# modelscope/FunCodec

Hardware: AMD Instinct MI355X
Metric: audio-seconds encoded+decoded per wall-sec, 16k-nq32ds640 (higher is better)
Workload: dtype f32; 1 GPU; BASELINE.json configs[1]: encodec 16k-nq32ds640 (57.6M, synthetic seeded checkpoint), run_mod=inference (encode + 32-stage RVQ + decode), 16 x 10 s utterances per GPU in micro-batches of 16, n_q=32; utterances_per_gpu=16, samples_per_utterance=160000, micro_batch=16, global_utterances=16, ranks_seen=1, parallelism=single GPU

## Files before the change

funcodec_amd/build.py:

```python
from __future__ import annotations

import concurrent.futures
import glob
import os
import shutil
import subprocess

HERE = os.path.dirname(os.path.abspath(__file__))
CSRC = os.path.join(HERE, "csrc")
LIB_PATH = os.path.join(HERE, "libfuncodec_amd.so")
OBJ_DIR = os.path.join(CSRC, "_obj")
HEADERS = ["kernels.h", "device_common.h", "conv_kernel.h", "laura_kernels.h", "seq_kernels.h", "stream_kernels.h", "ragged_kernels.h", "slots_kernels.h", os.path.join("..", "..", "include", "funcodec_amd.h")]


def sources():
    tiles = sorted(os.path.basename(p) for p in glob.glob(os.path.join(CSRC, "conv_tile*_*.hip")))
    heavy = [t for t in tiles if t.startswith("conv_tileq_") and "_m" not in t] + [t for t in tiles if t.endswith("_m01.hip")]
    rest = [t for t in tiles if t not in heavy]
    return heavy + ["kernels.hip", "laura_persist.hip", "laura_kernels.hip", "freq_kernels.hip", "seq_kernels.hip", "seqstream_kernels.hip", "stream_kernels.hip", "ragged_kernels.hip", "slots_kernels.hip", "engine.hip", "laura.hip"] + rest


def _hipcc() -> str:
    for cand in (os.environ.get("HIPCC"), shutil.which("hipcc"), "/opt/rocm/bin/hipcc"):
        if cand and os.path.exists(cand):
            return cand
    raise RuntimeError("hipcc not found")


def needs_build() -> bool:
    if not os.path.exists(LIB_PATH):
        return True
    t = os.path.getmtime(LIB_PATH)
    deps = [os.path.join(CSRC, s) for s in sources() + HEADERS]
    return any(os.path.exists(d) and os.path.getmtime(d) > t for d in deps)


def build(force: bool = False, verbose: bool = False) -> str:
    timeline = bool(os.environ.get("FC_TIMELINE"))
    out = LIB_PATH.replace(".so", "_timeline.so") if timeline else LIB_PATH
    defines = ["-DFC_TIMELINE", "-DFC_AB_KNOBS"] if timeline else []
    defines += ["-D" + f for f in os.environ.get("FC_BUILD_DEFINES", "").split()]
    if os.environ.get("FC_BUILD_OUT"):
        out = os.environ["FC_BUILD_OUT"]
    if not force and not defines and out == LIB_PATH and not needs_build():
        return LIB_PATH
    import hashlib
    hipcc = _hipcc()
    base = [hipcc, "--offload-arch=gfx950", "-O3", "-std=c++17", "-fPIC"] + defines
    tag = "".join(c if c.isalnum() else "_" for c in os.path.basename(out)) + "_" + hashlib.sha1(" ".join(base[1:]).encode()).hexdigest()[:10]
    obj_dir = os.path.join(OBJ_DIR, tag)
    os.makedirs(obj_dir, exist_ok=True)
    hdr_time = max(os.path.getmtime(os.path.join(CSRC, h)) for h in HEADERS if os.path.exists(os.path.join(CSRC, h)))

    def compile_one(src: str) -> str:
        obj = os.path.join(obj_dir, src.replace(".hip", ".o"))
        path = os.path.join(CSRC, src)
        if not force and os.path.exists(obj) and os.path.getmtime(obj) > max(os.path.getmtime(path), hdr_time):
            return obj
        cmd = base + ["-c", path, "-o", obj]
        if verbose:
            print(" ".join(cmd), flush=True)
        subprocess.run(cmd, check=True)
        return obj

    srcs = sources()
    with concurrent.futures.ThreadPoolExecutor(max_workers=min(len(srcs), os.cpu_count() or 4)) as ex:
        objs = list(ex.map(compile_one, srcs))
    tmp_out = f"{out}.{os.getpid()}.tmp"
    link = [hipcc, "--offload-arch=gfx950", "-shared", "-fPIC", "-o", tmp_out] + objs
    if verbose:
        print(" ".join(link), flush=True)
    subprocess.run(link, check=True)
# ... 7 lines not shown
```

funcodec_amd/csrc/engine.hip:

```cpp
#include <hip/hip_runtime.h>

#include <algorithm>
#include <array>
#include <cmath>
#include <cstdio>
#include <cstring>
#include <map>
#include <memory>
#include <string>
#include <vector>

#include "../../include/funcodec_amd.h"
#include "kernels.h"
#include "laura_kernels.h"
#include "ragged_kernels.h"
#include "seq_kernels.h"
#include "slots_kernels.h"
#include "stream_kernels.h"

namespace {

thread_local std::string g_err;

int fail(const std::string& msg) { g_err = msg; return 1; }
// ... 178 lines not shown
    ~Session() { drop_graphs(); }
};

struct fc_stream : Session {
    int enc_pushes = 0, dec_pushes = 0;
    int enc_frames = 0, dec_frames = 0;
    bool enc_done = false;
    bool broken = false;
};

struct fc_slots : Session {
    enum Phase : char { Idle, Running, Ended, Poisoned };
    std::vector<char> enc_phase, dec_phase;
    int enc_pushes = 0, dec_pushes = 0;
    std::vector<int32_t> push;
    std::vector<int32_t> enc_frames, dec_frames;
};

namespace {

hipEvent_t prof_event(fc_engine* e) {
    if (e->events_used == e->event_pool.size()) {
        hipEvent_t ev;
        if (hipEventCreate(&ev) != hipSuccess) return nullptr;
        e->event_pool.push_back(ev);
    }
    return e->event_pool[e->events_used++];
}

struct ProfSpan {
    fc_engine* e; hipStream_t st; int idx = -1;
    template <typename Cls>
    ProfSpan(fc_engine* e_, hipStream_t st_, bool live, Cls&& cls, double flops, double bytes) : e(e_), st(st_) {
        if (!e->profiling || !live) return;
        fc_engine::Span s; s.cls = e->prof_class(cls()); s.a = prof_event(e); s.b = prof_event(e); s.flops = flops; s.bytes = bytes;
        if (!s.a || !s.b) return;
        (void)hipEventRecord(s.a, st);
        e->spans.push_back(s);
        idx = (int)e->spans.size() - 1;
    }
    ~ProfSpan() { if (idx >= 0) (void)hipEventRecord(e->spans[idx].b, st); }
};

struct Ctx {
    fc_engine* e = nullptr;
    int B = 0;
    hipStream_t st = nullptr;
    char* base = nullptr;
    size_t cap = 0, off = 256;
    bool dry = false;
    int err = 0;
    bool dec_side = false, no_xq = false;
    int rate = 1;
    static constexpr size_t kTailSlack = 4096;
    int launches = 0, conv_launches = 0;
    double conv_flops = 0, conv_bytes = 0, lstm_flops = 0, rvq_flops = 0, attn_flops = 0;
    bool live() const { return !dry && !err; }
    void fail(const std::string& msg) {
        if (!err) { err = 1; g_err = msg; }
    }
    template <typename T>
    T* alloc(size_t n) {
        off = (off + 255) & ~(size_t)255;
        T* p = dry ? nullptr : (T*)(base + off);
        off += n * sizeof(T);
        if (!dry && off + kTailSlack > cap) { fail("workspace too small (sizes from fc_engine_workspace_bytes include 4 KiB of tail slack)"); return nullptr; }
        return p;
    }
    template <typename Enqueue>
    void launch(const char* what, const char* layer, Enqueue&& enqueue) {
        ++launches;
        if (live()) check(enqueue(), what, layer);
    }
    template <typename Cls, typename Enqueue>
    void launch(const char* what, const char* layer, Cls&& cls, double flops, double bytes, Enqueue&& enqueue) {
        ++launches;
        if (!live()) return;
        ProfSpan sp(e, st, true, cls, flops, bytes);
        check(enqueue(), what, layer);
    }
    template <typename Cls, typename Enqueue>
    void conv_launch(const char* what, const char* layer, Cls&& cls, double flops, double bytes, Enqueue&& enqueue) {
        ++conv_launches;
        launch(what, layer, cls, flops, bytes, enqueue);
    }
    void check(hipError_t er, const char* what, const char* layer) {
        if (er != hipSuccess) fail(std::string(what) + " launch failed" + (*layer ? std::string(" (") + layer + ")" : "") + ": " + hipGetErrorString(er));
    }
};

Ctx make_ctx(fc_engine* e, int B, void* ws, size_t ws_bytes, void* stream) {
    Ctx cx;
    cx.e = e; cx.B = B; cx.st = (hipStream_t)stream; cx.base = (char*)ws; cx.cap = ws_bytes;
    return cx;
}

Ctx dry_ctx(fc_engine* e, int B) {
    Ctx cx = make_ctx(e, B, nullptr, 0, nullptr);
    cx.dry = true;
    return cx;
}

template <typename T>
T* at(T* p, long long off) { return p ? p + off : nullptr; }

enum class Role { First, Shortcut, Block1, Block3, Resample, Last };
// ... 760 lines not shown
        cx.launch("halo rows", L.prefix.c_str(),
                  [&] { return fc::launch_halo_rows(halo_of->buf, cx.B, halo_of->F, halo_of->halo, halo_of->C, halo_of->T, 0, cx.st); });
}

Act run_conv(fc_engine* e, Ctx& cx, const ConvLayer& L, fc::Src s0, fc::Src s1, int elu, int Tin,
             float* out_override = nullptr, long long sB = 0, long long sM = 0, long long sT = 0) {
    const ConvGeom g = conv_geom(L, Tin);
    const bool has_prologue = (s0.used & 2) || s1.used || elu;
    int xq_Tp = 0;
    if ((L.Mpad / L.BM >= 3 || L.force_plain) && has_prologue) {
        const bool xq = !cx.no_xq && !s0.div && !out_override_blocks_xq(L) && fc::conv_xq_ok(L.cin, L.CC, L.gk, L.gstride, L.dil, L.BM, L.BN, L.row ? 1 : 0);
        const int padL_x = L.transposed ? 1 : g.padL, padR_x = L.transposed ? 1 : g.padR;
        const int Tp = padL_x + Tin + padR_x;
        float* tmp = xq ? cx.alloc<float>(fc::conv_xq_floats(cx.B, L.cin, Tp, L.BN, L.gstride, L.gk, L.dil))
                        : cx.alloc<float>((size_t)cx.B * L.cin * Tin);
        cx.launch("combine", L.prefix.c_str(), [&] {
            return xq ? fc::launch_combine_xq(s0, s1, elu, e->arch.elu_alpha, cx.B, L.cin, Tin, padL_x, padR_x, (L.transposed || L.zpadL >= 0) ? 1 : 0, tmp, cx.st)
                      : fc::launch_combine(s0, s1, elu, e->arch.elu_alpha, nullptr, cx.B, L.cin, Tin, Tin, tmp, (long long)L.cin * Tin, Tin, 1, cx.st);
        });
        s0 = fc::Src(); s0.ptr = tmp; s0.used = 1;
        s1 = fc::Src();
        elu = 0;
        if (xq) xq_Tp = Tp;
    }
    fc::ConvLaunch c = conv_launch_of(L, cx.B, Tin, g);
    c.s0 = s0; c.s1 = s1; c.elu = elu; c.alpha = e->arch.elu_alpha;
    c.xq_Tp = xq_Tp;
    Act out;
    out.C = L.cout; out.T = g.Tout;
    if (L.transposed) {
        c.Tout = Tin + 1; c.pad_zero = 1;
        c.up_r = L.stride; c.trimL = L.causal ? 0 : L.stride - L.stride / 2; c.Tfinal = g.Tout;
    } else {
        c.Tout = g.Tout;
        if (L.zpadL >= 0) c.pad_zero = 1;
    }
    if (out_override) {
        out.raw = out_override;
        c.out_sB = sB; c.out_sM = sM; c.out_sT = sT;
    } else {
        out.raw = cx.alloc<float>((size_t)cx.B * L.cout * g.Tout);
        c.out_sB = (long long)L.cout * g.Tout; c.out_sM = g.Tout; c.out_sT = 1;
    }
    c.out = out.raw;
    const int nblk = fc::conv_nblk(c);
    if (L.has_norm) {
        c.partials = cx.alloc<double>((size_t)cx.B * nblk * 2);
        out.aff = cx.alloc<float>((size_t)cx.B * L.cout * 2);
        out.normed = true;
    }
    const double fl = 2.0 * cx.B * (double)L.M * L.cin * L.gk * c.Tout;
    const double by = 4.0 * cx.B * ((double)L.cin * Tin * (s1.used ? 2 : 1) + (double)L.cout * g.Tout);
    cx.conv_flops += fl; cx.conv_bytes += by;
    cx.conv_launch("conv", L.prefix.c_str(), [&] { return conv_class(c); }, fl, by, [&] { return fc::launch_conv(c, cx.st); });
    conv_finish(e, cx, L, c.partials, nblk, (double)L.cout * g.count_T, out.aff);
    return out;
}

inline fc::Src src_of(const Act& a) { fc::Src s; s.ptr = a.raw; s.aff = a.aff; s.used = a.normed ? 3 : 1; s.ld = a.ld; return s; }

Act run_lstm(fc_engine* e, Ctx& cx, const LstmBlock& lb, const Act& in, int T, float* carried = nullptr, const fc::RagLen* steps = nullptr) {
    const int H = lb.H, B = cx.B, L = (int)lb.layers.size();
    float* xproj = cx.alloc<float>((size_t)T * B * 4 * H);
    run_conv(e, cx, lb.layers[0].inproj, src_of(in), fc::Src(), 0, T, xproj, (long long)4 * H, 1, (long long)B * 4 * H);
    static const int persist_env = fc::deploy_switch("FC_LSTM_PERSIST", 1);
    bool persist = false;
    if (!carried && persist_env && e->lstm_persist_ok) {
        const int key = B * 4096 + H;
        if (e->persist_checked_B != key) { e->persist_checked_val = fc::lstm_persist_supported(B, H, L, e->device); e->persist_checked_B = key; }
        persist = e->persist_checked_val;
    }
    const size_t BH = (size_t)B * H;
    float* state = carried ? carried : cx.alloc<float>(persist ? fc::lstm_persist_state_floats(B, H, T) : 3 * L * BH);
    Act y;
    y.C = H; y.T = T;
    y.raw = cx.alloc<float>((size_t)B * H * T);
    const double fl = 2.0 * B * (double)T * 4 * H * H * (2 * L - 1);
    cx.lstm_flops += fl;
    const double by = 4.0 * (4.0 * H * H * (2 * L - 1) + (double)T * B * 4.0 * H + (double)B * H * T);
    const float* w[FC_LSTM_MAX_LAYERS] = {nullptr};
    const float* bias[FC_LSTM_MAX_LAYERS] = {nullptr};
    for (int l = 0; l < L; ++l) { w[l] = l == 0 ? lb.layers[0].whh : lb.layers[l].wcat; bias[l] = lb.layers[l].bperm; }
    const char* pre = lb.prefix.c_str();
    ProfSpan sp(e, cx.st, cx.live(), [&] { return persist ? kLstmPersistClass : kLstmWaveClass; }, fl, by);
    if (!carried)
        cx.launch("lstm state clear", pre,
                  [&] { return fc::launch_zero_fill(state, persist ? fc::lstm_persist_clear_floats(B, H) : 3 * L * BH, cx.st); });
    if (persist) {
        cx.launch("lstm", pre, [&] { return fc::launch_lstm_persist(w[0], w[1], bias[1], xproj, state, y.raw, B, H, T, e->status_dev, cx.st); });
    } else {
        for (int s = 0; s < T + L - 1; ++s)
            cx.launch("lstm step", pre, [&] {
                return steps ? fc::launch_lstm_wave(w, bias, xproj, state, state + 2 * L * BH, y.raw, B, H, T, L, s, cx.st, steps->lens, steps->div, steps->mul)
                             : fc::launch_lstm_wave(w, bias, xproj, state, state + 2 * L * BH, y.raw, B, H, T, L, s, cx.st);
            });
    }
    if (carried && (T & 1))
        for (int l = 0; l < L; ++l)
            cx.launch("lstm carry", pre, [&] {
                return hipMemcpyAsync(state + (size_t)(2 * l + 1) * BH, state + (size_t)(2 * l) * BH, BH * sizeof(float), hipMemcpyDeviceToDevice, cx.st);
            });
    return y;
}

struct TfCache {
    float* base = nullptr;
// ... 167 lines not shown
}

void run_bottleneck(fc_engine* e, Ctx& cx, const Pass& p, bool dec, const Act& x, fc::Src* a0, fc::Src* a1) {
    const LstmBlock& lb = dec ? e->dec_lstm : e->enc_lstm;
    const TfBlock& tb = dec ? e->dec_tf : e->enc_tf;
    *a0 = src_of(x); *a1 = fc::Src();
    if (!has_seq(lb, tb)) return;
    Act y;
    switch (p.kind) {
        case Pass::Stream:
            if (tb.C) {
                const TfCache kv = tf_cache(*p.sess, dec, dec ? static_cast<const fc_stream*>(p.sess)->dec_frames : static_cast<const fc_stream*>(p.sess)->enc_frames);
                if (!cx.dry && kv.pos + x.T > p.sess->max_frames) { cx.fail("internal: a push past max_frames reached the transformer"); return; }
                y = run_transformer(e, cx, tb, x, x.T, &kv);
            } else {
                y = run_lstm(e, cx, lb, x, x.T, lstm_state(*p.sess, dec));
            }
            break;
        case Pass::Slots: {
            const fc::RagLen steps = ragged_len(cx, p);
            if (tb.C) {
                TfCache kv = tf_cache(*p.sess, dec, 0);
                kv.rows = true; kv.len = steps; kv.pos_dev = p.pos;
                if (p.host_push) { kv.host_len = p.host_push; kv.host_pos = p.host_push + 2 * cx.B; }
                kv.grid_bound = p.graphed;
                y = run_transformer(e, cx, tb, x, x.T, &kv);
            } else {
                y = run_lstm(e, cx, lb, x, x.T, lstm_state(*p.sess, dec), &steps);
            }
            break;
        }
        case Pass::Ragged:
        case Pass::Offline: y = run_seq(e, cx, lb, tb, x, x.T); break;
    }
    *a0 = src_of(y);
    if (e->arch.lstm_skip) *a1 = src_of(x);
}

void run_resblocks(fc_engine* e, Ctx& cx, const Pass& p, const fc_engine::Stage& S, fc::Src a0, fc::Src a1, int T, Act* sc, Act* b3) {
    for (const auto& R : S.res) {
        Act b1;
        if (p.kind == Pass::Offline && R.fused_head && !a0.div) {
            run_reshead(e, cx, R, a0, a1, T, sc, &b1);
        } else {
            *sc = walk_conv(e, cx, p, Role::Shortcut, R.shortcut, a0, a1, 0, T);
            b1 = walk_conv(e, cx, p, Role::Block1, R.block1, a0, a1, 1, T);
        }
        *b3 = walk_conv(e, cx, p, Role::Block3, R.block3, src_of(b1), fc::Src(), 1, b1.T);
        a0 = src_of(*sc); a1 = src_of(*b3);
    }
}

Act run_encoder(fc_engine* e, Ctx& cx, const Pass& p, fc::Src wav, int T) {
    cx.dec_side = false; cx.rate = 1; cx.no_xq = p.kind == Pass::Ragged;
    Act x = walk_conv(e, cx, p, Role::First, e->enc_first, wav, fc::Src(), 0, T);
    for (auto& S : e->enc_stages) {
        Act sc, b3;
        run_resblocks(e, cx, p, S, src_of(x), fc::Src(), x.T, &sc, &b3);
        x = walk_conv(e, cx, p, Role::Resample, S.resample, src_of(sc), src_of(b3), 1, sc.T);
        cx.rate *= S.resample.stride;
    }
    fc::Src a0, a1;
    run_bottleneck(e, cx, p, false, x, &a0, &a1);
    return walk_conv(e, cx, p, Role::Last, e->enc_last, a0, a1, 1, x.T);
}

Act run_decoder(fc_engine* e, Ctx& cx, const Pass& p, const float* z_bdt, int Tf) {
    fc::Src s; s.ptr = z_bdt; s.used = 1;
    cx.dec_side = true; cx.rate = 1; cx.no_xq = p.kind == Pass::Ragged;
    Act x = walk_conv(e, cx, p, Role::First, e->dec_first, s, fc::Src(), 0, Tf);
    fc::Src a0, a1;
    run_bottleneck(e, cx, p, true, x, &a0, &a1);
    int T = Tf;
    for (auto& S : e->dec_stages) {
        Act up = walk_conv(e, cx, p, Role::Resample, S.resample, a0, a1, 1, T);
        cx.rate *= S.resample.stride;
        Act sc, b3;
        run_resblocks(e, cx, p, S, src_of(up), fc::Src(), up.T, &sc, &b3);
        a0 = src_of(sc); a1 = src_of(b3);
        T = up.T;
    }
    return walk_conv(e, cx, p, Role::Last, e->dec_last, a0, a1, 1, T);
}



Act2 materialise2d(fc_engine* e, Ctx& cx, const ConvLayer& L, const Act2& x0, const Act2* x1, int elu, int pad) {
    const int B = cx.B, C = L.c2d;
    Act2 m;
    m.C = C; m.F = x0.F; m.T = x0.T; m.halo = x0.halo;
    m.buf = cx.alloc<float>((size_t)B * (m.F + 2 * m.halo) * C * m.T);
    const bool fuse_halo = !pad && halo_fuse_on() && m.F > m.halo;
    cx.launch("combine2d", L.prefix.c_str(), [&] {
        if (x0.halo < pad) return hipErrorInvalidValue;
        return fc::launch_combine2d(x0.buf, x0.aff, x0.halo, x1 ? x1->buf : nullptr, x1 ? x1->aff : nullptr, x1 ? x1->halo : 0, elu, e->arch.elu_alpha,
                                    B, m.F, C, m.T, m.buf, m.halo, cx.st, fuse_halo ? 1 : 0);
    });
    if (pad) cx.launch("halo rows", L.prefix.c_str(), [&] { return fc::launch_halo_rows_short(m.buf, B, m.F, m.halo, pad, C, m.T, cx.st); });
    else if (!fuse_halo) cx.launch("halo rows", L.prefix.c_str(), [&] { return fc::launch_halo_rows(m.buf, B, m.F, m.halo, C, m.T, 0, cx.st); });
    return m;
}

Act2 run_conv2d(fc_engine* e, Ctx& cx, const ConvLayer& L, Act2 x0, const Act2* x1, int elu, int out_halo) {
    const int B = cx.B, C = L.c2d, kf = L.kf, sf = L.sf;
    const int tot_f = (kf - 1) - (sf - 1), f_after = tot_f / 2, f_before = tot_f - f_after;
    const int Fo = (x0.F + tot_f - kf) / sf + 1;
    const ConvGeom g = conv_geom(L, x0.T);
    const int fpad = std::max(f_before, f_after);
    if (x0.F <= fpad) { x0 = materialise2d(e, cx, L, x0, x1, elu, fpad); x1 = nullptr; elu = 0; }
    bool mat;
    if (L.w_group) {
        static const int gmat = fc::ab_knob("FC_GCONV_MAT", 1);
        mat = gmat && kf >= 4 && x1;
    } else {
        static const int few_mat = fc::ab_knob("FC_FEWOUT_MAT", 1);
        const bool few_out = few_mat && L.cout <= 4 && L.stride == 1 && sf == 1 && (L.k == 3 || L.k == 5 || L.k == 7) && kf > 1;
        mat = (L.Mpad / L.BM >= 3 || few_out || L.force_plain) && (x0.normed || x1 || elu);
    }
    if (mat) { x0 = materialise2d(e, cx, L, x0, x1, elu, 0); x1 = nullptr; elu = 0; }
    Act2 o;
    o.C = L.cout; o.F = Fo; o.T = g.Tout; o.halo = out_halo;
    o.buf = cx.alloc<float>((size_t)B * (Fo + 2 * out_halo) * L.cout * g.Tout);
// ... 1439 lines not shown
    return cx.err;
}
}

int fc_freq_synthesis_size(const fc_engine* ce, int B, int C, int F, int Tp, int out_len, size_t* workspace_bytes) {
    fc_engine* e = const_cast<fc_engine*>(ce);
    if (freq_synthesis_check(e, B, C, F, Tp, out_len)) return 1;
    if (!workspace_bytes) return fail("null argument");
    Ctx cx = dry_ctx(e, B);
    if (freq_synthesis(e, cx, nullptr, nullptr, nullptr, Tp, out_len, nullptr, nullptr)) return 1;
    *workspace_bytes = cx.off + 4096;
    return 0;
}

int fc_freq_synthesis(fc_engine* e, const float* dec, const float* aff, const float* scale, int B, int C, int F, int Tp, int out_len, float* wav,
                      float* spec, void* workspace, size_t workspace_bytes, void* stream) {
    if (freq_synthesis_check(e, B, C, F, Tp, out_len)) return 1;
    if (!dec || !wav) return fail("bad argument");
    if (check_ready(e)) return 1;
    Ctx cx = make_ctx(e, B, workspace, workspace_bytes, stream);
    return freq_synthesis(e, cx, dec, aff, scale, Tp, out_len, wav, spec);
}

namespace {
fc::Src hook_src(const float* x, const float* aff, const float* div) {
    fc::Src s;
    s.ptr = x; s.aff = aff; s.div = div;
    s.used = x ? ((aff || div) ? 3 : 1) : 0;
    return s;
}
}

static int layer_src_check(const fc_engine* e, const char* prefix, const float* x0, const float* aff0, const float* div0, const float* x1,
                           const float* aff1, int B, int T, const ConvLayer** out) {
    if (!e || !prefix || !x0 || B <= 0 || T <= 0 || (aff1 && !x1) || (aff0 && div0)) return fail("bad argument");
    auto it = e->by_prefix.find(prefix);
    if (it == e->by_prefix.end()) return fail(std::string("unknown layer ") + prefix);
    const ConvLayer& L = *it->second;
    if (L.c2d > 0)
        return fail(std::string("layer ") + prefix + " is a 2-D layer of the STFT-domain codec: use fc_layer2d_forward");
    if (x1 && !L.dual) return fail("fc_layer_forward_src: " + L.prefix + " is planned for one source (its staging has no room for two)");
    if (div0 && &L != &e->enc_first) return fail("fc_layer_forward_src: div0 is the encoder's first conv's volume scale (" + e->enc_first.prefix + ")");
    *out = &L;
    return 0;
}

int fc_layer_forward_src(fc_engine* e, const char* prefix, const float* x0, const float* aff0, const float* div0, const float* x1,
                         const float* aff1, int B, int T, int apply_elu, float* y, void* workspace, size_t workspace_bytes, void* stream) {
    const ConvLayer* L = nullptr;
    if (layer_src_check(e, prefix, x0, aff0, div0, x1, aff1, B, T, &L)) return 1;
    if (!y) return fail("bad argument");
    if (check_ready(e)) return 1;
    Ctx cx = make_ctx(e, B, workspace, workspace_bytes, stream);
    Act o = run_conv(e, cx, *L, hook_src(x0, aff0, div0), hook_src(x1, aff1, nullptr), apply_elu, T);
    if (cx.err) return 1;
    HIP_TRY(fc::launch_combine(src_of(o), fc::Src(), 0, 1.f, nullptr, B, o.C, o.T, o.T, y, (long long)o.C * o.T, o.T, 1, cx.st));
    return 0;
}

int fc_layer_forward(fc_engine* e, const char* prefix, const float* x, int B, int T, int apply_elu, float* y,
                     void* workspace, size_t workspace_bytes, void* stream) {
    return fc_layer_forward_src(e, prefix, x, nullptr, nullptr, nullptr, nullptr, B, T, apply_elu, y, workspace, workspace_bytes, stream);
}

int fc_resblock_forward_src(fc_engine* e, const char* prefix, const float* x0, const float* aff0, const float* x1, const float* aff1, int B,
                            int T, float* y, void* workspace, size_t workspace_bytes, void* stream) {
    if (!e || !prefix || !x0 || !y || B <= 0 || T <= 0 || (aff1 && !x1)) return fail("bad argument");
    auto it = e->res_by_prefix.find(prefix);
    if (it == e->res_by_prefix.end()) return fail(std::string("unknown residual block ") + prefix);
    const fc_engine::ResBlock& R = *it->second;
    if (x1 && !R.shortcut.dual)
        return fail(std::string("fc_resblock_forward_src: block ") + prefix + " is planned for one source (its staging has no room for two)");
    if (check_ready(e)) return 1;
    Ctx cx = make_ctx(e, B, workspace, workspace_bytes, stream);
    fc_engine::Stage one;
    one.res.push_back(R);
    Act sc, b3;
    run_resblocks(e, cx, Pass(), one, hook_src(x0, aff0, nullptr), hook_src(x1, aff1, nullptr), T, &sc, &b3);
    if (cx.err) return 1;
    HIP_TRY(fc::launch_combine(src_of(sc), src_of(b3), 0, 1.f, nullptr, B, sc.C, T, T, y, (long long)sc.C * T, T, 1, cx.st));
    return 0;
}

int fc_resblock_forward(fc_engine* e, const char* prefix, const float* x, int B, int T, float* y, void* workspace,
                        size_t workspace_bytes, void* stream) {
    return fc_resblock_forward_src(e, prefix, x, nullptr, nullptr, nullptr, B, T, y, workspace, workspace_bytes, stream);
}

int fc_lstm_forward(fc_engine* e, const char* prefix, const float* x, int B, int T, float* y, void* workspace,
                    size_t workspace_bytes, void* stream) {
    if (check_ready(e)) return 1;
    if (!prefix || !x || !y || B <= 0 || T <= 0) return fail("bad argument");
    auto it = e->lstm_by_prefix.find(prefix);
    if (it == e->lstm_by_prefix.end()) return fail(std::string("unknown lstm ") + prefix);
    Ctx cx = make_ctx(e, B, workspace, workspace_bytes, stream);
    Act in; in.raw = const_cast<float*>(x); in.C = it->second->H; in.T = T;
    Act o = run_lstm(e, cx, *it->second, in, T);
    if (cx.err) return 1;
    fc::Src s1;
    if (e->arch.lstm_skip) s1 = src_of(in);
    HIP_TRY(fc::launch_combine(src_of(o), s1, 0, 1.f, nullptr, B, o.C, T, T, y, (long long)o.C * T, T, 1, cx.st));
    return 0;
}

int fc_seq_forward(fc_engine* e, const char* prefix, const float* x, int B, int T, float* y, void* workspace,
                   size_t workspace_bytes, void* stream) {
// ... 472 lines not shown
```

funcodec_amd/csrc/kernels.h:

```cpp
#pragma once
#include <hip/hip_runtime.h>
#include <stdint.h>
#include <stdio.h>
#include <stdlib.h>

#include <vector>

namespace fc {

inline int ab_knob(const char* name, int dflt) {
#ifdef FC_AB_KNOBS
    const char* v = getenv(name);
    return v ? atoi(v) : dflt;
#else
    if (getenv(name)) fprintf(stderr, "funcodec_amd: %s is set but ignored by this build (tuning knobs need FC_BUILD_DEFINES=FC_AB_KNOBS)\n", name);
    return dflt;
#endif
}

inline int deploy_switch(const char* name, int dflt) {
    const char* v = getenv(name);
    return v ? atoi(v) : dflt;
}

struct Src {
    const float* ptr = nullptr;
    const float* aff = nullptr;
    const float* div = nullptr;
    int used = 0;
    int ld = 0;
};

struct ConvLaunch {
    Src s0, s1;
    int elu = 0; float alpha = 1.f;
    const float* wt = nullptr;
    const float* bias = nullptr;
    const int* koff = nullptr;
    float* out = nullptr;
    long long out_sB = 0, out_sM = 0, out_sT = 1;
    int B = 0, Cin = 0, Tin = 0;
    int M = 0;
    int Tout = 0;
    int k = 1, stride = 1, padL = 0, padR = 0;
    int dil = 1;
    int pad_zero = 0;
    int up_r = 0, trimL = 0, Tfinal = 0;
    double* partials = nullptr;
    int BM = 128, BN = 128, CC = 2, nchunk = 1;
    int row = 0;
    int xq_Tp = 0;
    int Fo = 1;
    int affC = 0;
    long long in_sB0 = 0, in_sB1 = 0;
    long long out_sF = 0, part_sB0 = 0;
    int store_lo = 0, store_hi = 1 << 30;
    const float* w_plain = nullptr;
    float bias_host0 = 0.f;
};

int conv_nblk(const ConvLaunch& c);
bool conv_cout1_ok(const ConvLaunch& c);
bool conv_fewout_rows(const ConvLaunch& c);
void conv_fewout_name(const ConvLaunch& c, char* buf, size_t n);
size_t conv_lds_bytes(const ConvLaunch& c);
int conv_wbuf_floats(int k, int CC, int BM);
bool conv_quad(int CC);
size_t conv_pack_index(int k, int CC, int BM, int kk, int cl, int mm);
size_t conv_lds_bytes_for(int k, int stride, int dil, int CC, int BM, int BN, int Cin, int ntab, int row, int dma_rounds = -1);
bool conv_row_ok(int k, int stride, int dil, int CC, int BM, int BN, int Cin, bool dual);
bool conv_slab_fits(int k, int stride, int dil, int CC, int BN, int BM, bool dual);
int conv_wgs_per_cu(int BM);
std::vector<int> conv_koff_table(int k, int stride, int dil, int CC, int BN, int row);
hipError_t launch_conv(const ConvLaunch& c, hipStream_t st);
void conv_variant(const ConvLaunch& c, int* mode, int* nu, int* row);

struct ResHeadLaunch {
    Src s0, s1;
    const float *wsc = nullptr, *wb1 = nullptr;
    const float *bsc = nullptr, *bb1 = nullptr;
    float *out_sc = nullptr, *out_b1 = nullptr;
    double *part_sc = nullptr, *part_b1 = nullptr;
    int B = 0, C = 0, T = 0, k = 3, dil = 1, padL = 0, padR = 0;
    float alpha = 1.f;
};
bool reshead_ok(int C, int hid, int k_sc, int k_b1, int dil, int stride);
int reshead_ntiles(int T);
hipError_t launch_reshead(const ResHeadLaunch& c, hipStream_t st);

struct GConvLaunch {
    const float *src0 = nullptr, *aff0 = nullptr, *src1 = nullptr, *aff1 = nullptr;
    const float *w = nullptr, *bias = nullptr;
    float* out = nullptr;
    double* partials = nullptr;
    int B = 0, C = 0, M = 0, G = 1, Tin = 0, Tout = 0, Fo = 0, kf = 1, kt = 1, sf = 1, st = 1, padL = 0, padR = 0, elu = 0;
    float alpha = 1.f;
    long long in_sB = 0, in_sF = 0, out_sB = 0, out_sF = 0;
    const char *guard_lo = nullptr, *guard_hi = nullptr;
    int out_halo = 0;
};
bool gconv2d_ok(int cpg, int opg, int kf, int kt, int st);
bool gconv2d_fuses_halo(int kf, int kt, int st, int Fo, int halo);
int gconv2d_nblk(int Tout, int Fo, int G, int kf);
hipError_t launch_gconv2d(const GConvLaunch& c, hipStream_t st);
bool gconvtr2d_ok(int cpg, int opg, int tr);
int gconvtr2d_nblk(int Tin, int tr, int Fin, int fr);
hipError_t launch_gconvtr2d(const float* z, const float* w, const float* bias, float* out, double* partials, int B, int C, int cout, int Fin,
                            int Tin, int fr, int tr, int f_l, int Fout, int trimL, int Tout, long long out_sB, hipStream_t st,
                            int out_halo = 0 );
hipError_t launch_polyphase_in(const float* wav, const float* div, int B, int T, int hop, int n_fft, int Mp, float* xp, hipStream_t st);
hipError_t launch_stft_feats(const float* spec, int B, int F, int Tp, long long spec_sB, int halo, int C, float* feats, hipStream_t st);
hipError_t launch_feats_relayout(float* eng, float* ref, int B, int C, int F, int Tp, int halo, int to_ref, hipStream_t st);
hipError_t launch_halo_rows(float* buf, int B, int F, int halo, int C, int T, int zero, hipStream_t st);
hipError_t launch_halo_rows_short(float* buf, int B, int F, int halo, int pad, int C, int T, hipStream_t st);
hipError_t launch_combine2d(const float* s0, const float* aff0, int h0, const float* s1, const float* aff1, int h1, int elu, float alpha,
                            int B, int F, int C, int T, float* dst, int hd, hipStream_t st,
                            int halo_mode = 0 );
hipError_t launch_spec_from_dec(const float* dec, const float* aff, int B, int F, int Tp, int halo, int C, float* spec, hipStream_t st);
hipError_t launch_istft_finish(const float* ypoly, const float* win2, int B, int hop, int n_fft, int Mp, int Tp, const float* mul, int out_len,
                               float* wav, hipStream_t st);

hipError_t launch_gn_finalize(const double* partials, int nblk, double count, const float* gamma,
                              const float* beta, int C, float eps, int B, float* aff, hipStream_t st);

bool conv_xq_ok(int Cin, int CC, int k, int stride, int dil, int BM, int BN, int row);
size_t conv_xq_floats(int B, int Cin, int Tp, int BN, int stride, int k, int dil);
hipError_t launch_combine_xq(const Src& s0, const Src& s1, int elu, float alpha, int B, int C, int Tin, int padL, int padR, int pad_zero,
                             float* xq, hipStream_t st);
// ... 58 lines not shown
```

Before: 10660 audio-s/s.

## Add persistent MFMA kernel for thin 32/64-channel convolutions in offline passes

Adds a specialized conv kernel for the first strided downsampling conv (Cin=32, k=4, s=2) and the final transposed upsampling conv (Cin=64, k=2, up_r=2). The kernel keeps weights resident in LDS, double-buffers input slabs with buffer loads, fuses the affine-norm and ELU prologue, and loops over several tiles per workgroup with a persistent grid. It also writes GroupNorm partials and handles output trimming in the epilogue. It is only used for offline passes when the tile count times batch is large enough, which adds a large specialized code path and new edge-handling logic.

```diff
diff --git a/funcodec_amd/build.py b/funcodec_amd/build.py
--- a/funcodec_amd/build.py
+++ b/funcodec_amd/build.py
@@ -17,7 +17,7 @@
     tiles = sorted(os.path.basename(p) for p in glob.glob(os.path.join(CSRC, "conv_tile*_*.hip")))
     heavy = [t for t in tiles if t.startswith("conv_tileq_") and "_m" not in t] + [t for t in tiles if t.endswith("_m01.hip")]
     rest = [t for t in tiles if t not in heavy]
-    return heavy + ["kernels.hip", "laura_persist.hip", "laura_kernels.hip", "freq_kernels.hip", "seq_kernels.hip", "seqstream_kernels.hip", "stream_kernels.hip", "ragged_kernels.hip", "slots_kernels.hip", "engine.hip", "laura.hip"] + rest
+    return heavy + ["kernels.hip", "conv_thin2.hip", "laura_persist.hip", "laura_kernels.hip", "freq_kernels.hip", "seq_kernels.hip", "seqstream_kernels.hip", "stream_kernels.hip", "ragged_kernels.hip", "slots_kernels.hip", "engine.hip", "laura.hip"] + rest
 
 
 def _hipcc() -> str:
diff --git a/funcodec_amd/csrc/conv_thin2.hip b/funcodec_amd/csrc/conv_thin2.hip
--- /dev/null
+++ b/funcodec_amd/csrc/conv_thin2.hip
@@ -0,0 +1,445 @@
+#include "device_common.h"
+#include "kernels.h"
+
+#include <atomic>
+#include <type_traits>
+
+namespace fc {
+
+typedef float t2_f32x16 __attribute__((ext_vector_type(16)));
+typedef float t2_f32x2 __attribute__((ext_vector_type(2)));
+typedef float t2_f32x2u __attribute__((ext_vector_type(2), aligned(4)));
+
+__device__ __forceinline__ __amdgpu_buffer_rsrc_t t2_rsrc(const float* base) {
+    return __builtin_amdgcn_make_buffer_rsrc((void*)base, 0, 0x7fffffff, 0x00020000);
+}
+__device__ __forceinline__ f32x4 t2_ld4(__amdgpu_buffer_rsrc_t r, unsigned voff, int soff) {
+    return __builtin_bit_cast(f32x4, __builtin_amdgcn_raw_buffer_load_b128(r, (int)voff, soff, 0));
+}
+__device__ __forceinline__ float t2_ld1(__amdgpu_buffer_rsrc_t r, unsigned voff, int soff) {
+    return __builtin_bit_cast(float, __builtin_amdgcn_raw_buffer_load_b32(r, (int)voff, soff, 0));
+}
+typedef unsigned int t2_u32x2 __attribute__((ext_vector_type(2)));
+__device__ __forceinline__ void t2_st1(__amdgpu_buffer_rsrc_t r, unsigned voff, int soff, float v) {
+    __builtin_amdgcn_raw_buffer_store_b32(__builtin_bit_cast(unsigned, v), r, (int)voff, soff, 0);
+}
+__device__ __forceinline__ void t2_st2(__amdgpu_buffer_rsrc_t r, unsigned voff, int soff, float a, float b) {
+    __builtin_amdgcn_raw_buffer_store_b64((t2_u32x2){__builtin_bit_cast(unsigned, a), __builtin_bit_cast(unsigned, b)}, r, (int)voff, soff, 0);
+}
+
+__device__ __forceinline__ int t2_fresh_lane() {
+    int l;
+    asm volatile("v_mbcnt_lo_u32_b32 %0, -1, 0\n\tv_mbcnt_hi_u32_b32 %0, -1, %0" : "=v"(l));
+    return l;
+}
+
+struct Thin2Args {
+    const float *src0, *aff0, *src1, *aff1;
+    const float* wt;
+    const float* bias;
+    float* out;
+    double* partials;
+    long long out_sB, out_sM;
+    int Tin, Tout, padR, Leff, ntiles, trimL, Tfinal;
+    float alpha;
+};
+
+constexpr int T2_BN = 256;
+constexpr int T2_SLAB = 4160;
+constexpr int T2_W = 8192;
+
+template <bool TR, bool DUAL>
+__global__ __launch_bounds__(256, 2) void conv_thin2_kernel(const Thin2Args p) {
+    constexpr int CIN = TR ? 64 : 32;
+    constexpr int ICH = TR ? 16 : 8;
+    constexpr int NIT = CIN / ICH;
+    constexpr int RS = TR ? 260 : 520;
+    constexpr int LPR = TR ? 64 : 128;
+    constexpr int RSTEP = 256 / LPR;
+    constexpr int INW = TR ? 256 : 512;
+    constexpr int NHALO = 16;
+    extern __shared__ __attribute__((aligned(16))) float smem[];
+    float* Xs = smem;
+    float* Ws = Xs + 2 * T2_SLAB;
+    float2* tab0 = (float2*)(Ws + T2_W);
+    float2* tab1 = tab0 + 64;
+    float* bias_s = (float*)(tab1 + 64);
+    float2* red = (float2*)(bias_s + 64);
+
+    const int tid = threadIdx.x, lane = tid & 63, wid = __builtin_amdgcn_readfirstlane(tid >> 6);
+    const int hi = lane >> 5, l31 = lane & 31;
+    const int b = blockIdx.y;
+    const int t_begin = (int)(((long long)p.ntiles * blockIdx.x) / gridDim.x);
+    const int t_end = (int)(((long long)p.ntiles * (blockIdx.x + 1)) / gridDim.x);
+    if (t_begin >= t_end) return;
+
+    for (int i = tid * 4; i < T2_W; i += 1024) *(f32x4*)(Ws + i) = *(const f32x4*)(p.wt + i);
+    if (tid < 64) bias_s[tid] = p.bias[tid];
+    if (tid < CIN) {
+        tab0[tid] = p.aff0 ? ((const float2*)p.aff0)[(size_t)b * CIN + tid] : make_float2(1.f, 0.f);
+        tab1[tid] = (DUAL && p.aff1) ? ((const float2*)p.aff1)[(size_t)b * CIN + tid] : make_float2(1.f, 0.f);
+    }
+
+    const int c4 = tid & (LPR - 1), row0 = tid / LPR;
+    const bool has_h = tid < NHALO;
+    const int h_row = has_h ? (TR ? tid : tid >> 1) : 0;
+    const int h_side = (!TR && has_h) ? (tid & 1) : 0;
+    const int h_col = h_side ? INW : -1;
+    const size_t ubase = (size_t)b * CIN * p.Tin;
+    const float* s0 = p.src0 + ubase;
+    const float* s1 = DUAL ? p.src1 + ubase : s0;
+    const unsigned ld_voff = 4u * (unsigned)(row0 * p.Tin + 4 * c4 + 1);
+    const unsigned h_voff = has_h ? 4u * (unsigned)(h_row * p.Tin + h_col + 1) : 0u;
+    const unsigned st_voff = TR ? 4u * (unsigned)(2 * hi * (int)p.out_sM + 2 * (wid * 64 + l31)) : 4u * (unsigned)(4 * hi * (int)p.out_sM + wid * 64 + l31);
+    const int padL = 1;
+    const int refl = 2 * (p.Leff - 1), hi_lim = p.Tin + p.padR;
+    auto resolve = [&](int g, bool& ok) __attribute__((always_inline)) {
+        ok = g >= -padL && g < hi_lim;
+        int src = g < 0 ? -g : g;
+        src = src >= p.Leff ? refl - src : src;
+        if (TR) { src = g; ok = ok && g >= 0; }
+        ok = ok && src < p.Tin;
+        return ok ? src : 0;
+    };
+
+    f32x4 v0[2][4], v1[2][DUAL ? 4 : 1];
+    float hv0[2] = {0.f, 0.f}, hv1[2] = {0.f, 0.f};
+    unsigned vmask[2] = {0u, 0u};
+    auto load_item = [&](auto set_tag, auto fast_tag, int ld_tile, int ld_it) __attribute__((always_inline)) {
+        constexpr int S = decltype(set_tag)::value;
+        constexpr bool FAST = decltype(fast_tag)::value;
+        const int g0 = ld_tile * INW, c0 = ld_it * ICH;
+        if (FAST) {
+            const size_t org = (size_t)c0 * p.Tin + g0 - 1;
+            const __amdgpu_buffer_rsrc_t q0 = t2_rsrc(s0 + org), q1 = t2_rsrc(s1 + org);
+            const int row_b = 4 * RSTEP * p.Tin;
+#pragma unroll
+            for (int r = 0; r < 4; ++r) {
+                v0[S][r] = t2_ld4(q0, ld_voff, r * row_b);
+                if (DUAL) v1[S][r] = t2_ld4(q1, ld_voff, r * row_b);
+            }
+            hv0[S] = t2_ld1(q0, h_voff, 0);
+            if (DUAL) hv1[S] = t2_ld1(q1, h_voff, 0);
+        } else {
+            unsigned vm = 0, off[4];
+#pragma unroll
+            for (int j = 0; j < 4; ++j) {
+                bool ok;
+                off[j] = 4u * (unsigned)(row0 * p.Tin + resolve(g0 + 4 * c4 + j, ok));
+                vm |= (ok ? 1u : 0u) << j;
+            }
+            const __amdgpu_buffer_rsrc_t q0 = t2_rsrc(s0 + (size_t)c0 * p.Tin), q1 = t2_rsrc(s1 + (size_t)c0 * p.Tin);
+            const int row_b = 4 * RSTEP * p.Tin;
+#pragma unroll
+            for (int r = 0; r < 4; ++r)
+#pragma unroll
+                for (int j = 0; j < 4; ++j) {
+                    v0[S][r][j] = t2_ld1(q0, off[j], r * row_b);
+                    if (DUAL) v1[S][r][j] = t2_ld1(q1, off[j], r * row_b);
+                }
+            bool ok;
+            const unsigned hoff = 4u * (unsigned)(h_row * p.Tin + resolve(g0 + h_col, ok));
+            hv0[S] = t2_ld1(q0, hoff, 0);
+            if (DUAL) hv1[S] = t2_ld1(q1, hoff, 0);
+            vm |= (ok ? 1u : 0u) << 4;
+            vmask[S] = vm;
+        }
+    };
+    auto prologue = [&](float v, float w, float2 a, float2 a1) __attribute__((always_inline)) {
+        v = fmaf(v, a.x, a.y);
+        if (DUAL) v = v + fmaf(w, a1.x, a1.y);
+        return elu_f(v, p.alpha);
+    };
+    auto stage_item = [&](auto set_tag, auto fast_tag, float* Xd, int st_it) __attribute__((always_inline)) {
+        constexpr int S = decltype(set_tag)::value;
+        constexpr bool FAST = decltype(fast_tag)::value;
+        const int c0 = st_it * ICH;
+        const unsigned vm = FAST ? 0x1fu : vmask[S];
+        float2 a[4], a1[4];
+#pragma unroll
+        for (int r = 0; r < 4; ++r) { a[r] = tab0[c0 + row0 + RSTEP * r]; a1[r] = tab1[c0 + row0 + RSTEP * r]; }
+        const float2 ah = tab0[c0 + h_row], ah1 = tab1[c0 + h_row];
+#pragma unroll
+        for (int r = 0; r < 4; ++r) {
+            f32x4 x;
+#pragma unroll
+            for (int j = 0; j < 4; ++j) {
+                float v = prologue(v0[S][r][j], DUAL ? v1[S][r][j] : 0.f, a[r], a1[r]);
+                if (!FAST) v = ((vm >> j) & 1u) ? v : 0.f;
+                x[j] = v;
+            }
+            float* row = Xd + (row0 + RSTEP * r) * RS;
+            if (TR) {
+                *(f32x4*)(row + 4 + 4 * c4) = x;
+            } else {
+                *(t2_f32x2*)(row + 260 + 2 * c4) = (t2_f32x2){x[0], x[2]};
+                *(t2_f32x2*)(row + 2 + 2 * c4) = (t2_f32x2){x[1], x[3]};
+            }
+        }
+        {
+            float v = prologue(hv0[S], hv1[S], ah, ah1);
+            if (!FAST) v = ((vm >> 4) & 1u) ? v : 0.f;
+            const int h_idx = has_h ? h_row * RS + (TR ? 3 : (h_side ? 516 : 1)) : 0;
+            if (FAST) Xd[h_idx] = v;
+            else if (has_h) Xd[h_idx] = v;
+        }
+    };
+
+    t2_f32x16 acc[2][2];
+    auto init_acc = [&]() __attribute__((always_inline)) {
+        const int hi = t2_fresh_lane() >> 5;
+#pragma unroll
+        for (int i = 0; i < 2; ++i)
+#pragma unroll
+            for (int r = 0; r < 16; ++r) {
+                const float bias = bias_s[i * 32 + (r & 3) + 8 * (r >> 2) + 4 * hi];
+#pragma unroll
+                for (int j = 0; j < 2; ++j) acc[i][j][r] = bias;
+            }
+    };
+    auto flush_stats = [&](int tile) __attribute__((always_inline)) {
+        if (!p.partials || wid != 0) return;
+        const int lane = t2_fresh_lane();
+        const float2* r = red + (tile & 1) * 256;
+        double d1 = 0.0, d2 = 0.0;
+#pragma unroll
+        for (int j = 0; j < 4; ++j) { const float2 v = r[lane + 64 * j]; d1 += (double)v.x; d2 += (double)v.y; }
+#pragma unroll
+        for (int o = 32; o >= 1; o >>= 1) {
+            d1 += __shfl_xor(d1, o, 64);
+            d2 += __shfl_xor(d2, o, 64);
+        }
+        if (lane == 0) {
+            const size_t slot_p = ((size_t)b * p.ntiles + tile) * 2;
+            p.partials[slot_p] = d1;
+            p.partials[slot_p + 1] = d2;
+        }
+    };
+    auto epilogue = [&](int tile, auto fast_tag) __attribute__((always_inline)) {
+        constexpr bool FAST = decltype(fast_tag)::value;
+        const int n0 = tile * T2_BN;
+        const int nb = n0 + wid * 64 + l31;
+        float s1v = 0.f, s2v = 0.f;
+        float* ob = p.out + (size_t)b * (size_t)p.out_sB;
+        if (!TR) {
+            const bool full = FAST || n0 + T2_BN <= p.Tout;
+            const __amdgpu_buffer_rsrc_t qo = t2_rsrc(ob + n0);
+            const int sMb = 4 * (int)p.out_sM;
+#pragma unroll
+            for (int i = 0; i < 2; ++i)
+#pragma unroll
+                for (int r = 0; r < 16; ++r)
+#pragma unroll
+                    for (int j = 0; j < 2; ++j) {
+                        if (!FAST && !full && nb + j * 32 >= p.Tout) continue;
+                        const float v = acc[i][j][r];
+                        s1v += v;
+                        s2v = fmaf(v, v, s2v);
+                        t2_st1(qo, st_voff, (i * 32 + (r & 3) + 8 * (r >> 2)) * sMb + j * 128, v);
+                    }
+        } else {
+#pragma unroll
+            for (int i = 0; i < 2; ++i)
+#pragma unroll
+                for (int r = 0; r < 16; ++r)
+#pragma unroll
+                    for (int j = 0; j < 2; ++j) {
+                        if (!FAST && nb + j * 32 >= p.Tout) continue;
+                        const float v = acc[i][j][r];
+                        s1v += v;
+                        s2v = fmaf(v, v, s2v);
+                    }
+            if (FAST) {
+                const __amdgpu_buffer_rsrc_t qo = t2_rsrc(ob + 2 * n0 - p.trimL);
+                const int sMb = 4 * (int)p.out_sM;
+#pragma unroll
+                for (int i = 0; i < 2; ++i)
+#pragma unroll
+                    for (int rq = 0; rq < 4; ++rq)
+#pragma unroll
+                        for (int j = 0; j < 2; ++j) {
+                            t2_st2(qo, st_voff, (i * 16 + 4 * rq) * sMb + j * 256, acc[i][j][4 * rq], acc[i][j][4 * rq + 1]);
+                            t2_st2(qo, st_voff, (i * 16 + 4 * rq + 1) * sMb + j * 256, acc[i][j][4 * rq + 2], acc[i][j][4 * rq + 3]);
+                        }
+            } else {
+                const __amdgpu_buffer_rsrc_t qo = t2_rsrc(ob);
+                const int sMb = 4 * (int)p.out_sM;
+                const unsigned rowv = 4u * (unsigned)(2 * hi * (int)p.out_sM);
+#pragma unroll
+                for (int i = 0; i < 2; ++i)
+#pragma unroll
+                    for (int rq = 0; rq < 4; ++rq)
+#pragma unroll
+                        for (int j = 0; j < 2; ++j) {
+                            const int n = nb + j * 32;
+                            if (n >= p.Tout) continue;
+                            const float a0 = acc[i][j][4 * rq], a1 = acc[i][j][4 * rq + 1], a2 = acc[i][j][4 * rq + 2], a3 = acc[i][j][4 * rq + 3];
+                            const int t = 2 * n - p.trimL, so = (i * 16 + 4 * rq) * sMb;
+                            if (t >= 0 && t < p.Tfinal) { t2_st1(qo, rowv + 4u * (unsigned)t, so, a0); t2_st1(qo, rowv + 4u * (unsigned)t, so + sMb, a2); }
+                            if (t + 1 >= 0 && t + 1 < p.Tfinal) { t2_st1(qo, rowv + 4u * (unsigned)(t + 1), so, a1); t2_st1(qo, rowv + 4u * (unsigned)(t + 1), so + sMb, a3); }
+                        }
+            }
+        }
+        if (p.partials) red[(tile & 1) * 256 + wid * 64 + t2_fresh_lane()] = make_float2(s1v, s2v);
+    };
+
+    using Set0 = std::integral_constant<int, 0>;
+    using Set1 = std::integral_constant<int, 1>;
+    const f32x4* WsA = (const f32x4*)Ws + hi * 64 + l31;
+    const int xb_off = (TR ? hi * 4 * RS + 3 : (hi ? 260 : 1)) + wid * 64 + l31;
+    int flush_tile = -1;
+    __syncthreads();
+    init_acc();
+
+    auto mfma_item = [&](const float* Xd, int it) __attribute__((always_inline)) {
+        const float* Xb = Xd + xb_off;
+        if (!TR) {
+#pragma unroll
+            for (int cl = 0; cl < 2; ++cl) {
+                const f32x4* wa = WsA + (2 * it + cl) * 256;
+#pragma unroll
+                for (int q = 0; q < 2; ++q) {
+                    const f32x4 a0 = wa[q * 128], a1 = wa[q * 128 + 32];
+#pragma unroll
+                    for (int s4 = 0; s4 < 4; ++s4)
+#pragma unroll
+                        for (int j = 0; j < 2; ++j) {
+                            const float bv = Xb[(4 * cl + s4) * RS + j * 32 + q];
+                            acc[0][j] = __builtin_amdgcn_mfma_f32_32x32x2f32(a0[s4], bv, acc[0][j], 0, 0, 0);
+                            acc[1][j] = __builtin_amdgcn_mfma_f32_32x32x2f32(a1[s4], bv, acc[1][j], 0, 0, 0);
+                        }
+                }
+            }
+        } else {
+            const f32x4* wa = WsA + it * 512;
+#pragma unroll
+            for (int q = 0; q < 4; ++q) {
+                const f32x4 a0 = wa[q * 128], a1 = wa[q * 128 + 32];
+#pragma unroll
+                for (int s4 = 0; s4 < 4; ++s4)
+#pragma unroll
+                    for (int j = 0; j < 2; ++j) {
+                        const float bv = Xb[(8 * (q & 1) + s4) * RS + j * 32 + (q >> 1)];
+                        acc[0][j] = __builtin_amdgcn_mfma_f32_32x32x2f32(a0[s4], bv, acc[0][j], 0, 0, 0);
+                        acc[1][j] = __builtin_amdgcn_mfma_f32_32x32x2f32(a1[s4], bv, acc[1][j], 0, 0, 0);
+                    }
+            }
+        }
+    };
+    auto item = [&](int tile, int tb, auto it_tag, auto fast_tag) __attribute__((always_inline)) {
+        constexpr int IT = decltype(it_tag)::value;
+        constexpr bool FAST = decltype(fast_tag)::value;
+        using Set = std::integral_constant<int, IT & 1>;
+        float* Xd = Xs + (IT & 1) * T2_SLAB;
+        stage_item(Set(), fast_tag, Xd, IT);
+        __builtin_amdgcn_sched_barrier(0);
+        const int nt = IT < 2 ? tile : tile + 1;
+        if (FAST) load_item(Set(), fast_tag, nt < tb ? nt : tb - 1, (IT + 2) & 3);
+        else if (nt < tb) load_item(Set(), fast_tag, nt, (IT + 2) & 3);
+        __syncthreads();
+        if (IT == 0 && flush_tile >= 0) { flush_stats(flush_tile); flush_tile = -1; }
+        __builtin_amdgcn_sched_barrier(0);
+        mfma_item(Xd, IT);
+        __builtin_amdgcn_sched_barrier(0);
+    };
+    auto run = [&](int ta, int tb, auto fast_tag) __attribute__((always_inline)) {
+        if (ta >= tb) return;
+        __syncthreads();
+        if (flush_tile >= 0) { flush_stats(flush_tile); flush_tile = -1; }
+        load_item(Set0(), fast_tag, ta, 0);
+        load_item(Set1(), fast_tag, ta, 1);
+        for (int tile = ta; tile < tb; ++tile) {
+            item(tile, tb, std::integral_constant<int, 0>(), fast_tag);
+            item(tile, tb, std::integral_constant<int, 1>(), fast_tag);
+            item(tile, tb, std::integral_constant<int, 2>(), fast_tag);
+            item(tile, tb, std::integral_constant<int, 3>(), fast_tag);
+            epilogue(tile, fast_tag);
+            init_acc();
+            __builtin_amdgcn_sched_barrier(0);
+            flush_tile = tile;
+        }
+    };
+    constexpr int RIGHT = TR ? 0 : 1;
+    const int e0 = t_begin > 1 ? t_begin : 1;
+    const int e1 = p.Tin - RIGHT - INW >= 0 ? (p.Tin - RIGHT - INW) / INW + 1 : 0;
+    const int f0 = e0 > t_end ? t_end : e0;
+    const int f1 = e1 < f0 ? f0 : (e1 > t_end ? t_end : e1);
+    run(t_begin, f0, std::false_type());
+    run(f0, f1, std::true_type());
+    run(f1, t_end, std::false_type());
+    __syncthreads();
+    if (flush_tile >= 0) flush_stats(flush_tile);
+}
+
+static size_t thin2_lds_bytes() { return (size_t)(T2_W + 2 * T2_SLAB + 2 * 64 * 2 + 64 + 2 * 256 * 2) * sizeof(float); }
+
+int conv_thin2_switch() {
+    static const int v = deploy_switch("FC_THIN2", 1);
+    return v;
+}
+
+bool conv_thin2_ok(const ConvLaunch& c) {
+    if (!c.elu || c.s0.div || c.xq_Tp > 0 || c.Fo > 1 || c.out_sT != 1 || c.dil != 1 || c.in_sB0 || c.in_sB1 ||
+        (c.affC && c.affC != c.Cin) || c.store_lo != 0 || c.store_hi < 1)
+        return false;
+    if (c.M != 64 || c.BM != 64 || c.BN != 256 || !conv_quad(c.CC) || c.padL != 1 || c.Tin < 1) return false;
+    if ((unsigned long long)c.Cin * (unsigned long long)c.Tin * 4ull >= (1ull << 31)) return false;
+    if (c.out_sM <= 0 || (unsigned long long)c.out_sM * 64ull * 4ull >= (1ull << 31)) return false;
+    if (!c.up_r)
+        return c.Cin == 32 && c.k == 4 && c.stride == 2 && c.CC == 4 && c.nchunk == 8 && !c.row && !c.pad_zero && c.padR >= 1 &&
+               conv_wbuf_floats(c.k, c.CC, c.BM) == 1024;
+    return c.up_r == 2 && c.Cin == 64 && c.k == 2 && c.stride == 1 && c.CC == 16 && c.nchunk == 4 && c.row && c.pad_zero && c.Tout == c.Tin + 1 &&
+           c.trimL >= 0 && c.trimL <= 2 && c.Tfinal == 2 * c.Tin && conv_wbuf_floats(c.k, c.CC, c.BM) == 2048;
+}
+
+static int thin2_ntiles(const ConvLaunch& c) { return (c.Tout + T2_BN - 1) / T2_BN; }
+
+bool conv_thin2_takes(const ConvLaunch& c) {
+    const int sw = conv_thin2_switch();
+    if (sw == 0 || !conv_thin2_ok(c)) return false;
+    return sw >= 2 || (long long)thin2_ntiles(c) * c.B >= 512;
+}
+
+void conv_thin2_name(const ConvLaunch& c, char* buf, size_t n) {
+    snprintf(buf, n, "conv_thin2_kernel<%d, %d, %s, %s>", c.Cin, c.up_r ? c.M / 2 : c.M, c.up_r ? "true" : "false", c.s1.ptr ? "true" : "false");
+}
+
+template <bool TR, bool DUAL>
+static hipError_t launch_thin2_t(const Thin2Args& a, dim3 grid, hipStream_t st) {
+    static std::atomic<unsigned long long> attr_done{0ull};
+    auto kfn = conv_thin2_kernel<TR, DUAL>;
+    int dev = 0;
+    (void)hipGetDevice(&dev);
+    const unsigned long long bit = 1ull << (dev & 63);
+    if (!(attr_done.load(std::memory_order_acquire) & bit)) {
+        hipError_t ea = hipFuncSetAttribute((const void*)kfn, hipFuncAttributeMaxDynamicSharedMemorySize, 160 * 1024);
+        if (ea != hipSuccess) return ea;
+        attr_done.fetch_or(bit, std::memory_order_release);
+    }
+    hipLaunchKernelGGL(kfn, grid, dim3(256), thin2_lds_bytes(), st, a);
+    return hipGetLastError();
+}
+
+hipError_t launch_conv_thin2(const ConvLaunch& c, hipStream_t st) {
+    if (!conv_thin2_ok(c)) return hipErrorInvalidValue;
+    Thin2Args a;
+    a.src0 = c.s0.ptr; a.aff0 = c.s0.aff; a.src1 = c.s1.ptr; a.aff1 = c.s1.aff;
+    a.wt = c.wt; a.bias = c.bias; a.out = c.out; a.partials = c.partials;
+    a.out_sB = c.out_sB; a.out_sM = c.out_sM;
+    a.Tin = c.Tin; a.Tout = c.Tout; a.padR = c.padR;
+    const int maxpad = c.padL > c.padR ? c.padL : c.padR;
+    a.Leff = c.Tin > maxpad ? c.Tin : maxpad + 1;
+    a.ntiles = thin2_ntiles(c);
+    a.trimL = c.trimL; a.Tfinal = c.Tfinal;
+    a.alpha = c.alpha;
+    static const int target_env = deploy_switch("FC_TARGET_WGS", 0);
+    int G = (target_env ? target_env : 512) / c.B;
+    if (G < 1) G = 1;
+    if (G > a.ntiles) G = a.ntiles;
+    const dim3 grid(G, c.B);
+    const bool tr = c.up_r != 0, dual = c.s1.ptr != nullptr;
+    if (tr) return dual ? launch_thin2_t<true, true>(a, grid, st) : launch_thin2_t<true, false>(a, grid, st);
+    return dual ? launch_thin2_t<false, true>(a, grid, st) : launch_thin2_t<false, false>(a, grid, st);
+}
+
+}
diff --git a/funcodec_amd/csrc/engine.hip b/funcodec_amd/csrc/engine.hip
--- a/funcodec_amd/csrc/engine.hip
+++ b/funcodec_amd/csrc/engine.hip
@@ -254,6 +254,7 @@
     int err = 0;
     bool dec_side = false, no_xq = false;
     int rate = 1;
+    bool offline = false;
     static constexpr size_t kTailSlack = 4096;
     int launches = 0, conv_launches = 0;
     double conv_flops = 0, conv_bytes = 0, lstm_flops = 0, rvq_flops = 0, attn_flops = 0;
@@ -1120,6 +1121,16 @@
     const double fl = 2.0 * cx.B * (double)L.M * L.cin * L.gk * c.Tout;
     const double by = 4.0 * cx.B * ((double)L.cin * Tin * (s1.used ? 2 : 1) + (double)L.cout * g.Tout);
     cx.conv_flops += fl; cx.conv_bytes += by;
+    if (cx.offline && fc::conv_thin2_takes(c)) {
+        auto cls = [&] {
+            char nm[80];
+            fc::conv_thin2_name(c, nm, sizeof(nm));
+            return std::string(nm);
+        };
+        cx.conv_launch("conv", L.prefix.c_str(), cls, fl, by, [&] { return fc::launch_conv_thin2(c, cx.st); });
+        conv_finish(e, cx, L, c.partials, nblk, (double)L.cout * g.count_T, out.aff);
+        return out;
+    }
     cx.conv_launch("conv", L.prefix.c_str(), [&] { return conv_class(c); }, fl, by, [&] { return fc::launch_conv(c, cx.st); });
     conv_finish(e, cx, L, c.partials, nblk, (double)L.cout * g.count_T, out.aff);
     return out;
@@ -1393,7 +1404,7 @@
 }
 
 Act run_encoder(fc_engine* e, Ctx& cx, const Pass& p, fc::Src wav, int T) {
-    cx.dec_side = false; cx.rate = 1; cx.no_xq = p.kind == Pass::Ragged;
+    cx.dec_side = false; cx.rate = 1; cx.no_xq = p.kind == Pass::Ragged; cx.offline = p.kind == Pass::Offline;
     Act x = walk_conv(e, cx, p, Role::First, e->enc_first, wav, fc::Src(), 0, T);
     for (auto& S : e->enc_stages) {
         Act sc, b3;
@@ -1408,7 +1419,7 @@
 
 Act run_decoder(fc_engine* e, Ctx& cx, const Pass& p, const float* z_bdt, int Tf) {
     fc::Src s; s.ptr = z_bdt; s.used = 1;
-    cx.dec_side = true; cx.rate = 1; cx.no_xq = p.kind == Pass::Ragged;
+    cx.dec_side = true; cx.rate = 1; cx.no_xq = p.kind == Pass::Ragged; cx.offline = p.kind == Pass::Offline;
     Act x = walk_conv(e, cx, p, Role::First, e->dec_first, s, fc::Src(), 0, Tf);
     fc::Src a0, a1;
     run_bottleneck(e, cx, p, true, x, &a0, &a1);
@@ -2954,6 +2965,7 @@
     if (!y) return fail("bad argument");
     if (check_ready(e)) return 1;
     Ctx cx = make_ctx(e, B, workspace, workspace_bytes, stream);
+    cx.offline = true;
     Act o = run_conv(e, cx, *L, hook_src(x0, aff0, div0), hook_src(x1, aff1, nullptr), apply_elu, T);
     if (cx.err) return 1;
     HIP_TRY(fc::launch_combine(src_of(o), fc::Src(), 0, 1.f, nullptr, B, o.C, o.T, o.T, y, (long long)o.C * o.T, o.T, 1, cx.st));
diff --git a/funcodec_amd/csrc/kernels.h b/funcodec_amd/csrc/kernels.h
--- a/funcodec_amd/csrc/kernels.h
+++ b/funcodec_amd/csrc/kernels.h
@@ -74,6 +74,11 @@
 std::vector<int> conv_koff_table(int k, int stride, int dil, int CC, int BN, int row);
 hipError_t launch_conv(const ConvLaunch& c, hipStream_t st);
 void conv_variant(const ConvLaunch& c, int* mode, int* nu, int* row);
+
+bool conv_thin2_ok(const ConvLaunch& c);
+bool conv_thin2_takes(const ConvLaunch& c);
+void conv_thin2_name(const ConvLaunch& c, char* buf, size_t n);
+hipError_t launch_conv_thin2(const ConvLaunch& c, hipStream_t st);
 
 struct ResHeadLaunch {
     Src s0, s1;
```

After: 10680 audio-s/s (median of 6 runs). No clear change (+0.2%).
